# yoseph007/PQA2

Hardware: AMD Instinct MI355X
Metric: VMAF frames/sec (vif+adm+motion2 -> SVM), device-resident synthetic YUV pairs (higher is better)
Workload: dtype f32; 1 GPU; 2160p 3840x2160 8-bit, vmaf_4k_v0.6.1, 300 frames/GPU; frames_per_gpu=300, frames_total=300, batch=97, frames_per_launch=75, clips_pipelined=True, parallelism=frame-shard x1, 1-frame motion halo, all-gather of records + of scores

## Files before the change

pqa2_amd/csrc/kernels.h:

```cpp
#pragma once
#include <hip/hip_runtime.h>
#include <stdint.h>

namespace pqa {

enum Elem : int { ELEM_U8 = 0, ELEM_U16 = 1, ELEM_F32 = 2 };

struct PlaneRun {
  const void* base;
  int64_t row_pitch;
  int64_t frame_pitch;
};

struct MutPlaneRun {
  void* base;
  int64_t row_pitch;
  int64_t frame_pitch;
};

int vif_tile_w(int scale);
constexpr int kVifTileH = 8;
inline int vif_tiles_x(int scale, int w) { return (w + vif_tile_w(scale) - 1) / vif_tile_w(scale); }
inline int vif_tiles_y(int h) { return (h + kVifTileH - 1) / kVifTileH; }

enum : int { VIF_S0_VALU = 0, VIF_S0_AUTO = 1 };
hipError_t launch_vif_stat(hipStream_t stream, int scale, Elem elem, PlaneRun ref, PlaneRun dis, int n_frames,
                           int w, int h, float inv_scale, float gain_limit, int border101, double* partials,
                           MutPlaneRun next_ref, MutPlaneRun next_dis, int s0_mode = VIF_S0_AUTO, int* n_partials = nullptr);
hipError_t vif_march_prepare();
int vif_march_partials_max(int w, int h);
int vif_march_table(uint16_t* out, int capacity_halfwords);
void vif_march_shape(int w, int h, int* out6);
bool launch_vif_s0_march(hipStream_t stream, Elem elem, int bits, PlaneRun ref, PlaneRun dis, int n_frames, int w, int h, float gain_limit,
                         int border101, double* partials, MutPlaneRun next_ref, MutPlaneRun next_dis, int* n_partials,
                         hipError_t* err);
constexpr int kVifFxPartials = 8;
void vif_fixed_log2_table(uint16_t* out32768);
hipError_t launch_vif_fixed(hipStream_t stream, int scale, int bit_depth, Elem elem, PlaneRun ref, PlaneRun dis,
                            int n_frames, int w, int h, double gain_limit, const uint16_t* log2_lut,
                            long long* partials, MutPlaneRun next_ref, MutPlaneRun next_dis);

constexpr int kAdmTileW = 60, kAdmTileH = 14;
inline int adm_tiles_x(int band_w) { return (band_w + kAdmTileW - 1) / kAdmTileW; }
inline int adm_tiles_y(int band_h) { return (band_h + kAdmTileH - 1) / kAdmTileH; }

enum : int { ADM_TILED = 0, ADM_AUTO = 1, ADM_MARCH = 2 };
hipError_t launch_adm_scale(hipStream_t stream, int scale, Elem elem, PlaneRun ref, PlaneRun dis, int n_frames,
                            int w, int h, float inv_scale, float gain_limit, MutPlaneRun ll_ref,
                            MutPlaneRun ll_dis, double* partials, int mode = ADM_AUTO, int* n_partials = nullptr);
int adm_march_partials(int band_w, int band_h);
bool launch_adm_march(hipStream_t stream, int scale, Elem elem, PlaneRun ref, PlaneRun dis, int n_frames, int w, int h,
                      float inv_scale, float gain_limit, MutPlaneRun ll_ref, MutPlaneRun ll_dis, double* partials,
                      int* n_partials, hipError_t* err);
bool adm_pyramid_takes(Elem elem, int w, int h);
int adm_pyramid_partials(int w, int h);
bool launch_adm_pyramid(hipStream_t stream, Elem elem, PlaneRun ref, PlaneRun dis, int n_frames, int w, int h, float inv_scale,
                        float gain_limit, MutPlaneRun ll_ref, MutPlaneRun ll_dis, double* partials0, double* partials1,
                        int* n_partials, hipError_t* err);
float adm_dwt_quant_step(int lambda, int theta);

constexpr int kAdmFxRows = kAdmTileH + 2;
// ... 110 lines not shown
```

pqa2_amd/csrc/pqa_api.hip:

```cpp
#include "../../include/pqa_vmaf.h"

#include <algorithm>
#include <atomic>
#include <condition_variable>
#include <cstdarg>
#include <cstdio>
#include <cstdlib>
#include <cstring>
#include <memory>
#include <mutex>
#include <string>
#include <thread>
#include <vector>

#include <cerrno>
#include <unistd.h>

#include "host_pack.h"
#include "host_ring.h"
#include "ingest.h"
#include "kernels.h"

using namespace pqa;
using pqa::host::PackPool;
// ... 103 lines not shown
  uint8_t* luma_dev[2] = {nullptr, nullptr};
  hipEvent_t luma_copied[2] = {nullptr, nullptr};
  int64_t luma_pitch = 0;
  int LB = 0;
  bool luma_ready = false;
  uint32_t luma_gray = PQA_GRAY_LUMA;
  uint8_t* last_luma = nullptr;
  int64_t last_luma_pitch = 0;
  int64_t last_index = -1;
  bool have_last = false, halo_armed = false;
  Half half[2];
  int cur_half = 0, pending = 0;
  int64_t pending_first = 0;
  size_t slot_bytes = 0;
  size_t plane_off[2][3] = {};
  int64_t slot_row_pitch[3] = {};
  bool staging_ready = false;
  std::thread pin_thread;
  hipError_t pin_err = hipSuccess;
  uint8_t* surf_dev = nullptr;
  std::unique_ptr<PackPool> pack_pool;
  bool pack_pool_tried = false;
  std::vector<PackTask> pack_tasks;
  host::RecordRing ring;
  hipEvent_t batch_ev[kBatchEvents] = {};
  uint64_t batch_ev_seq[kBatchEvents] = {};
  uint64_t batch_seq = 0;
  uint64_t done_seq = 0;
  std::atomic<int> cancelled{0};
  std::string err;
  std::vector<void*> allocs;
  int multi_stream = 0;
  int vif_s0_mode = VIF_S0_AUTO;
  int adm_mode = ADM_AUTO;
  int motion_mode = MOTION_AUTO;
  bool trace = false;
  bool prof = false;
  uint32_t prof_mask = 0xffffffffu;
  std::vector<ProfEv> evs;
  double prof_ms[PQA_PROF_KERNELS] = {};
  uint64_t prof_n[PQA_PROF_KERNELS] = {}, prof_frames[PQA_PROF_KERNELS] = {};
};

namespace {

int fail(pqa_ctx* c, int code, const char* fmt, ...) {
  char buf[512];
  va_list ap;
  va_start(ap, fmt);
  vsnprintf(buf, sizeof buf, fmt, ap);
  va_end(ap);
  if (c) c->err = buf; else g_create_error = buf;
  return code;
}

#define HIPCHK(c, expr)                                                                          \
  do {                                                                                           \
    hipError_t e_ = (expr);                                                                      \
    if (e_ != hipSuccess)                                                                        \
      return fail((c), e_ == hipErrorOutOfMemory ? PQA_ENOMEM : PQA_EDEVICE, "%s failed: %s", #expr, \
                  hipGetErrorString(e_));                                                        \
  } while (0)

template <typename T>
int dev_alloc(pqa_ctx* c, T** out, size_t count) {
  void* p = nullptr;
// ... 134 lines not shown
      if (s < 3) {
        Level& L = c->vif_lv[s + 1];
        nr = MutPlaneRun{L.ref, L.pitch, L.frame_pitch};
        nd = MutPlaneRun{L.dis, L.pitch, L.frame_pitch};
      }
      {
        ProfScope ps(c, s, sp_n, st);
        HIPCHK(c, launch_vif_fixed(st, s, (int)c->cfg.bit_depth, ce, cr, cd, sp_n, cw, ch, c->cfg.vif_enhn_gain_limit,
                                   c->vif_lut, c->vif_fx_part[s], nr, nd));
      }
      if (s < 3) {
        Level& L = c->vif_lv[s + 1];
        cr = PlaneRun{L.ref, L.pitch, L.frame_pitch};
        cd = PlaneRun{L.dis, L.pitch, L.frame_pitch};
        ce = ELEM_U16;
        cw = L.w; ch = L.h;
      }
    }
  } else if ((feat & PQA_FEAT_VIF) && sp_n > 0) {
    PlaneRun cr = rYs, cd = dYs;
    Elem ce = c->elem;
    int cw = w, ch = h;
    for (int s = 0; s < 4; ++s) {
      MutPlaneRun nr{nullptr, 0, 0}, nd{nullptr, 0, 0};
      if (s < 3) {
        Level& L = c->vif_lv[s + 1];
        nr = MutPlaneRun{L.ref, L.pitch, L.frame_pitch};
        nd = MutPlaneRun{L.dis, L.pitch, L.frame_pitch};
      }
      {
        ProfScope ps(c, s, sp_n, st);
        HIPCHK(c, launch_vif_stat(st, s, ce, cr, cd, sp_n, cw, ch, c->inv_scale,
                                  (float)c->cfg.vif_enhn_gain_limit, c->cfg.vif_border == PQA_VIF_BORDER_INTEGER,
                                  c->vif_part[s], nr, nd, c->vif_s0_mode, &vif_np[s]));
      }
      if (s == 0 && fork_late) {
        HIPCHK(c, hipEventRecord(c->fork_ev, st));
        HIPCHK(c, hipStreamWaitEvent(st_adm, c->fork_ev, 0));
        HIPCHK(c, hipStreamWaitEvent(st_misc, c->fork_ev, 0));
      }
      if (s < 3) {
        Level& L = c->vif_lv[s + 1];
        cr = PlaneRun{L.ref, L.pitch, L.frame_pitch};
        cd = PlaneRun{L.dis, L.pitch, L.frame_pitch};
        ce = ELEM_F32;
        cw = L.w; ch = L.h;
      }
    }
  }
  if ((feat & PQA_FEAT_ADM) && sp_n > 0 && c->adm_fixed) {
    PlaneRun cr = rYs, cd = dYs;
    Elem ce = c->elem;
    int cw = w, ch = h;
    for (int s = 0; s < 4; ++s) {
      MutPlaneRun lr{nullptr, 0, 0}, ld{nullptr, 0, 0};
      if (s < 3) {
        Level& L = c->adm_lv[s + 1];
        lr = MutPlaneRun{L.ref, L.pitch, L.frame_pitch};
        ld = MutPlaneRun{L.dis, L.pitch, L.frame_pitch};
      }
      {
        ProfScope ps(c, 7 + s, sp_n, st_adm);
        HIPCHK(c, launch_adm_fixed(st_adm, s, (int)c->cfg.bit_depth, ce, cr, cd, sp_n, cw, ch,
                                   c->cfg.adm_enhn_gain_limit, c->adm_div_lut, lr, ld, c->adm_fx_part[s]));
      }
      if (s < 3) {
        Level& L = c->adm_lv[s + 1];
// ... 534 lines not shown
  c->k_sub = cfg->n_subsample > 1 ? (int)cfg->n_subsample : 1;
  if (c->cfg.vif_enhn_gain_limit <= 0) c->cfg.vif_enhn_gain_limit = 100.0;
  if (c->cfg.adm_enhn_gain_limit <= 0) c->cfg.adm_enhn_gain_limit = 100.0;
  c->elem = cfg->bit_depth > 8 ? ELEM_U16 : ELEM_U8;
  c->esize = cfg->bit_depth > 8 ? 2 : 1;
  c->inv_scale = 1.0f / (float)(1 << (cfg->bit_depth - 8));
  c->n_planes = (int)cfg->n_planes;
  c->pw[0] = (int)cfg->width; c->ph[0] = (int)cfg->height;
  for (int p = 1; p < 3; ++p) {
    c->pw[p] = (int)((cfg->width + (1u << cfg->chroma_hshift) - 1) >> cfg->chroma_hshift);
    c->ph[p] = (int)((cfg->height + (1u << cfg->chroma_vshift) - 1) >> cfg->chroma_vshift);
  }

  auto bail = [&](int rc) {
    g_create_error = c->err;
    pqa_destroy(c);
    return rc;
  };
#define CREATE_TRY(expr) do { int rc_ = (expr); if (rc_ != PQA_OK) return bail(rc_); } while (0)
#define CREATE_HIP(expr) do { hipError_t e_ = (expr); if (e_ != hipSuccess) { \
    fail(c, e_ == hipErrorOutOfMemory ? PQA_ENOMEM : PQA_EDEVICE, "%s failed: %s", #expr, hipGetErrorString(e_)); \
    return bail(e_ == hipErrorOutOfMemory ? PQA_ENOMEM : PQA_EDEVICE); } } while (0)

  CREATE_HIP(hipSetDevice(c->device));
  CREATE_HIP(hipStreamCreateWithFlags(&c->own_stream, hipStreamNonBlocking));
  c->stream = c->own_stream;
  {
    const char* e = getenv("PQA_MULTI_STREAM");
    c->multi_stream = (e && e[0] == '1') ? 1 : (e && e[0] == '2') ? 2 : 0;
    const char* t = getenv("PQA_TRACE");
    c->trace = t && t[0] == '1';
    const char* v = getenv("PQA_VIF_MFMA");
    c->vif_s0_mode = (v && v[0] == '0') ? VIF_S0_VALU : VIF_S0_AUTO;
    const char* am = getenv("PQA_ADM_MARCH");
    const char* ap = getenv("PQA_ADM_PYRAMID");
    c->adm_mode = (am && am[0] == '0') ? ADM_TILED : (ap && ap[0] == '0') ? ADM_MARCH : ADM_AUTO;
    const char* mm = getenv("PQA_MOTION_MARCH");
    c->motion_mode = (mm && mm[0] == '0') ? MOTION_TILED : MOTION_AUTO;
  }
  for (int i = 0; i < 2; ++i) {
    CREATE_HIP(hipStreamCreateWithFlags(&c->aux[i], hipStreamNonBlocking));
    CREATE_HIP(hipEventCreateWithFlags(&c->join_ev[i], hipEventDisableTiming));
  }
  CREATE_HIP(hipEventCreateWithFlags(&c->fork_ev, hipEventDisableTiming));
  for (int i = 0; i < kBatchEvents; ++i) CREATE_HIP(hipEventCreateWithFlags(&c->batch_ev[i], hipEventDisableTiming));
  try {
    c->ring.init(c->capacity);
  } catch (...) {
    fail(c, PQA_ENOMEM, "out of host memory");
    return bail(PQA_ENOMEM);
  }

  c->vif_fixed = (cfg->features & PQA_FEAT_VIF) && (cfg->fixed_point & PQA_FIXED_VIF);
  c->motion_fixed = (cfg->features & PQA_FEAT_MOTION) && (cfg->fixed_point & PQA_FIXED_MOTION);
  c->adm_fixed = (cfg->features & PQA_FEAT_ADM) && (cfg->fixed_point & PQA_FIXED_ADM);
  if (c->adm_fixed) {
    std::vector<int32_t> lut(65537);
    adm_fixed_div_table(lut.data());
    CREATE_TRY(dev_alloc(c, &c->adm_div_lut, lut.size()));
    CREATE_HIP(hipMemcpy(c->adm_div_lut, lut.data(), lut.size() * sizeof(int32_t), hipMemcpyHostToDevice));
  }
  if ((cfg->features & PQA_FEAT_VIF) && !c->vif_fixed) CREATE_HIP(vif_march_prepare());
  if (c->vif_fixed) {
    std::vector<uint16_t> lut(32768);
    vif_fixed_log2_table(lut.data());
    CREATE_TRY(dev_alloc(c, &c->vif_lut, lut.size()));
    CREATE_HIP(hipMemcpy(c->vif_lut, lut.data(), lut.size() * sizeof(uint16_t), hipMemcpyHostToDevice));
  }
  const int w = c->pw[0], h = c->ph[0], B = c->B;
  int vw = w, vh = h, aw = w, ah = h;
  for (int s = 0; s < 4; ++s) {
    if (s > 0) {
      vw /= 2; vh /= 2;
      aw = (aw + 1) / 2; ah = (ah + 1) / 2;
      Level& V = c->vif_lv[s];
      V.w = vw; V.h = vh; V.pitch = round_up(vw, 16); V.frame_pitch = V.pitch * vh;
      Level& A = c->adm_lv[s];
      A.w = aw; A.h = ah; A.pitch = round_up(aw, 16); A.frame_pitch = A.pitch * ah;
      if (cfg->features & PQA_FEAT_VIF) {
        CREATE_TRY(dev_alloc(c, &V.ref, (size_t)V.frame_pitch * B));
        CREATE_TRY(dev_alloc(c, &V.dis, (size_t)V.frame_pitch * B));
      }
      if (cfg->features & PQA_FEAT_ADM) {
        CREATE_TRY(dev_alloc(c, &A.ref, (size_t)A.frame_pitch * B));
        CREATE_TRY(dev_alloc(c, &A.dis, (size_t)A.frame_pitch * B));
      }
    }
    if (vw < 2 || vh < 2) { fail(c, PQA_EINVAL, "frame too small for 4 VIF scales"); return bail(PQA_EINVAL); }
    c->vif_tiles[s] = vif_tiles_x(s, vw) * vif_tiles_y(vh);
    if (s == 0) {
      const int mp = vif_march_partials_max(vw, vh);
      c->vif_part_cap0 = c->vif_tiles[0] > mp ? c->vif_tiles[0] : mp;
    }
    const int bw = (aw + 1) / 2, bh = (ah + 1) / 2;
    c->adm_tiles[s] = adm_tiles_x(bw) * adm_tiles_y(bh);
    const int left = (int)(bw * 0.1 - 0.5), top = (int)(bh * 0.1 - 0.5);
    c->adm_area[s] = (float)((bh - 2 * top) * (bw - 2 * left));
    if ((cfg->features & PQA_FEAT_VIF) && !c->vif_fixed)
      CREATE_TRY(dev_alloc(c, &c->vif_part[s], (size_t)(s == 0 ? c->vif_part_cap0 : c->vif_tiles[s]) * 2 * B));
    if ((cfg->features & PQA_FEAT_VIF) && c->vif_fixed)
      CREATE_TRY(dev_alloc(c, &c->vif_fx_part[s], (size_t)c->vif_tiles[s] * kVifFxPartials * B));
    c->adm_fx[s] = adm_fixed_scale_params(s, bw, bh);
    if ((cfg->features & PQA_FEAT_ADM) && !c->adm_fixed) {
      int mp = adm_march_partials(bw, bh);
      if (s < 2 && adm_pyramid_takes(c->elem, w, h)) { const int pp = adm_pyramid_partials(w, h); mp = pp > mp ? pp : mp; }
      CREATE_TRY(dev_alloc(c, &c->adm_part[s], (size_t)(c->adm_tiles[s] > mp ? c->adm_tiles[s] : mp) * 6 * B));
    }
    if ((cfg->features & PQA_FEAT_ADM) && c->adm_fixed)
      CREATE_TRY(dev_alloc(c, &c->adm_fx_part[s], (size_t)c->adm_tiles[s] * kAdmFxRows * 6 * B));
  }
  c->motion_tiles_n = motion_tiles(w, h);
  if (cfg->features & PQA_FEAT_MOTION) {
    {
      const int mp = motion_march_partials(w, h);
      CREATE_TRY(dev_alloc(c, &c->motion_part, (size_t)(c->motion_tiles_n > mp ? c->motion_tiles_n : mp) * B));
    }
    if (c->motion_fixed) CREATE_TRY(dev_alloc(c, &c->motion_fx_part, (size_t)c->motion_tiles_n * B));
    c->last_luma_pitch = round_up((int64_t)w * c->esize, 64);
    CREATE_TRY(dev_alloc(c, &c->last_luma, (size_t)c->last_luma_pitch * h));
  }
  for (int p = 0; p < c->n_planes; ++p) {
    if (cfg->features & PQA_FEAT_PSNR) {
      CREATE_TRY(dev_alloc(c, &c->sse_part[p], (size_t)kSseBlocksPerPlane * B));
      CREATE_TRY(dev_alloc(c, &c->sse_part_b[p], (size_t)kSseBlocksPerPlane * B));
    }
    if (cfg->features & PQA_FEAT_SSIM) {
      c->ssim_tiles_n[p] = ssim_tiles(c->pw[p], c->ph[p]);
      const int ww = (c->pw[p] >> 2) - 1, wh = (c->ph[p] >> 2) - 1;
      c->ssim_norm[p] = (ww > 0 && wh > 0) ? 1.0 / ((double)ww * wh) : 0.0;
      CREATE_TRY(dev_alloc(c, &c->ssim_part[p], (size_t)(c->ssim_tiles_n[p] ? c->ssim_tiles_n[p] : 1) * B));
      CREATE_TRY(dev_alloc(c, &c->sse_tile_part[p], (size_t)(c->ssim_tiles_n[p] ? c->ssim_tiles_n[p] : 1) * B));
    }
// ... 578 lines not shown
```

pqa2_amd/csrc/vif.hip:

```cpp
#include <cstring>
#include <mutex>
#include <vector>

#include <cstdio>
#include "kernels.h"
#include "pqa_device.h"

namespace pqa {

namespace {

struct Taps {
  float f[17];
};

static Taps gaussian_taps(int n) {
  Taps t{};
  double v[17], sum = 0.0;
  const double sigma = n / 5.0;
  for (int k = 0; k < n; ++k) {
    const double d = k - n / 2;
    v[k] = exp(-0.5 * d * d / (sigma * sigma));
    sum += v[k];
  }
  for (int k = 0; k < n; ++k) t.f[k] = (float)(v[k] / sum);
  return t;
}

struct TapPairs {
  f2 vt[18];
  f2 ht[17];
  f2 dt[9];
};

static TapPairs tap_pairs(const Taps& t, int n, const Taps* next, int n_next) {
  TapPairs p{};
  if (next)
    for (int k = 0; k < n_next; ++k) p.dt[k] = f2{next->f[k], next->f[k]};
  for (int k = 0; k <= n; ++k) {
    p.vt[k].x = k < n ? t.f[k] : 0.0f;
    p.vt[k].y = k > 0 ? t.f[k - 1] : 0.0f;
  }
  for (int k = 0; k < n; ++k) p.ht[k] = f2{t.f[k], t.f[k]};
  return p;
}

struct VifStatArgs {
  const void* ref;
  const void* dis;
  int64_t row_pitch_r, frame_pitch_r, row_pitch_d, frame_pitch_d;
  int w, h, tiles_x, n_tiles;
  int fold_w, fold_h;
  float inv_scale, gain_limit;
  double* partials;
  float* dst_ref;
  float* dst_dis;
  int64_t dst_row_pitch_r, dst_frame_pitch_r, dst_row_pitch_d, dst_frame_pitch_d;
  TapPairs taps;
};

constexpr int kP2 = 258;


template <int N, int TW, int ND>
__device__ __forceinline__ void vif_hstat(const VifStatArgs& a, const f2* sv ,
                                          const f2* sd , double* red, int fr, int tile, int x0, int y0) {
  constexpr int R = N / 2, TH = kVifTileH, NSEG = TW / 4, NRP = TH / 2;
  constexpr int RD = ND / 2;
  const int tid = threadIdx.x;
  fr = __builtin_amdgcn_readfirstlane(fr); tile = __builtin_amdgcn_readfirstlane(tile);
  x0 = __builtin_amdgcn_readfirstlane(x0); y0 = __builtin_amdgcn_readfirstlane(y0);
  if (ND) {
    const int ox0 = x0 >> 1, oy0 = y0 >> 1, ow = a.w >> 1, oh = a.h >> 1;
    float* __restrict__ tr = a.dst_ref + ((int64_t)fr * a.dst_frame_pitch_r + (int64_t)oy0 * a.dst_row_pitch_r + ox0);
    float* __restrict__ td = a.dst_dis + ((int64_t)fr * a.dst_frame_pitch_d + (int64_t)oy0 * a.dst_row_pitch_d + ox0);
    const unsigned rp_r = (unsigned)a.dst_row_pitch_r, rp_d = (unsigned)a.dst_row_pitch_d;
#pragma unroll
    for (int round = 0; round < 2; ++round) {
      const int item = tid + round * kBlock;
      const int oc = item & 127, orow = item >> 7;
      if (oc < TW / 2 && (ox0 + oc < ow && oy0 + orow < oh)) {
        f2 acc = f2{0.0f, 0.0f};
#pragma unroll
        for (int k = 0; k < ND; ++k) acc = __builtin_elementwise_fma(a.taps.dt[k], sd[orow * kP2 + 2 * oc + (R - RD) + k], acc);
        *reinterpret_cast<float*>(reinterpret_cast<char*>(tr) + ((unsigned)orow * rp_r + (unsigned)oc) * 4u) = acc.x;
        *reinterpret_cast<float*>(reinterpret_cast<char*>(td) + ((unsigned)orow * rp_d + (unsigned)oc) * 4u) = acc.y;
      }
    }
  }

  const int wave = tid >> 6, lane = tid & 63;
  const int rp = lane & 3, sl = lane >> 2;
  const int seg = 2 * (sl & 3) + (wave & 1) + 8 * (sl >> 2) + 32 * (wave >> 1);
  float num = 0.0f, den = 0.0f;
  if (seg < NSEG) {
    constexpr int NCOL = 4 + N - 1, NREAD = (NCOL + 1) / 2;
    f2 out[5][4];
#pragma unroll
    for (int s = 0; s < 5; ++s) {
      f2 in[2 * NREAD];
      const f4* p = reinterpret_cast<const f4*>(&sv[(s * NRP + rp) * kP2 + seg * 4]);
#pragma unroll
      for (int q = 0; q < NREAD; ++q) {
        const f4 v = p[q];
        in[2 * q] = f2{v.x, v.y};
        in[2 * q + 1] = f2{v.z, v.w};
      }
#pragma unroll
      for (int o = 0; o < 4; ++o) out[s][o] = f2{0.0f, 0.0f};
#pragma unroll
      for (int k = 0; k < N; ++k)
#pragma unroll
        for (int o = 0; o < 4; ++o) out[s][o] = __builtin_elementwise_fma(a.taps.ht[k], in[o + k], out[s][o]);
      __builtin_amdgcn_sched_barrier(0);
    }
    const float sigma_nsq = 2.0f, eps = 1.0e-10f, sigma_max_inv = 4.0f / (255.0f * 255.0f);
    const int gyA = y0 + 2 * rp;
    const bool vrow[2] = {gyA < a.h, gyA + 1 < a.h};
    f2 num2 = f2{0.0f, 0.0f}, den2 = f2{0.0f, 0.0f};
    f2 pn = f2{1.0f, 1.0f}, qn = f2{1.0f, 1.0f}, pd = f2{1.0f, 1.0f};
#pragma unroll
    for (int o = 0; o < 4; ++o) {
      const bool vcol = (x0 + seg * 4 + o) < a.w;
      const f2 mu1 = out[0][o], mu2 = out[1][o];
      const f2 s1 = out[2][o] - mu1 * mu1;
      f2 s2 = out[3][o] - mu2 * mu2;
      const f2 s12 = out[4][o] - mu1 * mu2;
      s2 = f2{fmaxf(s2.x, 0.0f), fmaxf(s2.y, 0.0f)};
      const bool vx = vcol && vrow[0], vy = vcol && vrow[1];
      const bool hx = vx && !(s1.x < sigma_nsq), hy = vy && !(s1.y < sigma_nsq);
      const bool lx = vx && (s1.x < sigma_nsq), ly = vy && (s1.y < sigma_nsq);
      const f2 s1h = f2{hx ? s1.x : 0.0f, hy ? s1.y : 0.0f};
      const f2 gden = s1h + f2{eps, eps};
      const f2 grcp = f2{fast_rcp(gden.x), fast_rcp(gden.y)};
      f2 g = s12 * grcp;
      g = __builtin_elementwise_fma(__builtin_elementwise_fma(-g, gden, s12), grcp, g);
      f2 sv = s2 - g * s12;
      sv = f2{fmaxf(sv.x, eps), fmaxf(sv.y, eps)};
      g = f2{__builtin_amdgcn_fmed3f(g.x, 0.0f, a.gain_limit), __builtin_amdgcn_fmed3f(g.y, 0.0f, a.gain_limit)};
      const f2 svn = sv + f2{sigma_nsq, sigma_nsq};
      const f2 narg = __builtin_elementwise_fma(g * g, s1h, svn);
      const f2 darg = __builtin_elementwise_fma(s1h, f2{1.0f / sigma_nsq, 1.0f / sigma_nsq}, f2{1.0f, 1.0f});
      const f2 low = __builtin_elementwise_fma(s2, f2{-sigma_max_inv, -sigma_max_inv}, f2{1.0f, 1.0f});
      pn *= narg;
      qn *= svn;
      pd *= darg;
      const f2 wl = f2{lx ? 1.0f : 0.0f, ly ? 1.0f : 0.0f};
      num2 = __builtin_elementwise_fma(wl, low, num2);
      den2 += wl;
      __builtin_amdgcn_sched_barrier(0);
    }
    num = (num2.x + num2.y) + ((fast_log2(pn.x) - fast_log2(qn.x)) + (fast_log2(pn.y) - fast_log2(qn.y)));
    den = (den2.x + den2.y) + (fast_log2(pd.x) + fast_log2(pd.y));
  }
  {
    const float part[2] = {num, den};
    double v[2];
    block_sum_f32<2>(part, v, red);
    if (tid == 0) {
      double* out = a.partials + ((int64_t)fr * a.n_tiles + tile) * 2;
      out[0] = v[0];
      out[1] = v[1];
    }
  }
}

template <typename T, int N, int TW, int ND>
__global__ __launch_bounds__(kBlock, 3) void vif_stat_kernel(const VifStatArgs a) {
  constexpr int R = N / 2, TH = kVifTileH, COLS = TW + N - 1, NSEG = TW / 4, S = 8, NIN = S + N - 1;
  constexpr int RD = ND / 2;
  static_assert(ND == 0 || RD <= R, "decimation window must sit inside the statistic window");
  static_assert(COLS <= 256 && COLS <= kP2, "one column per thread");
  static_assert(TW % 4 == 0 && NSEG <= 64 && TH == S, "segment map");
  __shared__ f2 sv[5][TH / 2][kP2];
  __shared__ f2 sd[ND ? TH / 2 : 1][ND ? kP2 : 1];
  __shared__ double red[12];

  const int tile = xcd_remap(blockIdx.x, a.n_tiles);
  const int tx = tile % a.tiles_x, ty = tile / a.tiles_x;
  const int fr = blockIdx.y;
  const T* __restrict__ ref = (const T*)a.ref + (int64_t)fr * a.frame_pitch_r;
  const T* __restrict__ dis = (const T*)a.dis + (int64_t)fr * a.frame_pitch_d;
  const int x0 = tx * TW, y0 = ty * TH;
  const int tid = threadIdx.x;

  {
    const int col = tid;
    constexpr int seg = 0;
    if (col < COLS) {
      const unsigned gx = (unsigned)mirror_fold(x0 - R + col, a.w, a.fold_w);
      const unsigned pitch_r = (unsigned)a.row_pitch_r, pitch_d = (unsigned)a.row_pitch_d;
      const auto rsrc_r = make_rsrc(ref, (unsigned)a.h * pitch_r * (unsigned)sizeof(T));
      const auto rsrc_d = make_rsrc(dis, (unsigned)a.h * pitch_d * (unsigned)sizeof(T));
      f2 acc[S / 2][5];
#pragma unroll
      for (int p = 0; p < S / 2; ++p)
// ... 61 lines not shown
        for (int s = 0; s < 5; ++s) sv[s][seg * (S / 2) + p][col] = acc[p][s];
      if (ND) {
#pragma unroll
        for (int q = 0; q < S / 2; ++q) sd[seg * (S / 2) + q][col] = dacc[q];
      }
    }
  }
  __syncthreads();

  vif_hstat<N, TW, ND>(a, &sv[0][0][0], &sd[0][0], red, fr, tile, x0, y0);
}


template <int N, int TW, int ND>
hipError_t launch_stat_n(hipStream_t stream, Elem elem, const VifStatArgs& a, int n_frames) {
  const dim3 grid(a.n_tiles, n_frames), block(kBlock);
  switch (elem) {
    case ELEM_U8: hipLaunchKernelGGL((vif_stat_kernel<uint8_t, N, TW, ND>), grid, block, 0, stream, a); break;
    case ELEM_U16: hipLaunchKernelGGL((vif_stat_kernel<uint16_t, N, TW, ND>), grid, block, 0, stream, a); break;
    case ELEM_F32: hipLaunchKernelGGL((vif_stat_kernel<float, N, TW, ND>), grid, block, 0, stream, a); break;
  }
  return hipGetLastError();
}

constexpr int kVifN[4] = {17, 9, 5, 3};
constexpr int kVifTW[4] = {240, 248, 252, 252};

}

int vif_tile_w(int scale) { return kVifTW[scale]; }

hipError_t launch_vif_stat(hipStream_t stream, int scale, Elem elem, PlaneRun ref, PlaneRun dis, int n_frames,
                           int w, int h, float inv_scale, float gain_limit, int border101, double* partials,
                           MutPlaneRun next_ref, MutPlaneRun next_dis, int s0_mode, int* n_partials) {
  if (n_partials) *n_partials = vif_tiles_x(scale, w) * vif_tiles_y(h);
  if (n_frames <= 0) return hipSuccess;
  const int bits = elem == ELEM_U8 ? 8 : (elem == ELEM_U16 && inv_scale == 0.25f) ? 10 : (elem == ELEM_U16 && inv_scale == 0.0625f) ? 12 : 0;
  if (scale == 0 && bits && s0_mode == VIF_S0_AUTO && next_ref.base && next_dis.base) {
    hipError_t err = hipSuccess;
    if (launch_vif_s0_march(stream, elem, bits, ref, dis, n_frames, w, h, gain_limit, border101, partials, next_ref, next_dis, n_partials, &err))
      return err;
    if (n_partials) *n_partials = vif_tiles_x(scale, w) * vif_tiles_y(h);
  }
  VifStatArgs a{};
  a.ref = ref.base; a.dis = dis.base;
  a.row_pitch_r = ref.row_pitch; a.frame_pitch_r = ref.frame_pitch;
  a.row_pitch_d = dis.row_pitch; a.frame_pitch_d = dis.frame_pitch;
  a.w = w; a.h = h;
  a.fold_w = 2 * w - (border101 ? 2 : 1); a.fold_h = 2 * h - (border101 ? 2 : 1);
  a.tiles_x = vif_tiles_x(scale, w);
  a.n_tiles = a.tiles_x * vif_tiles_y(h);
  a.inv_scale = inv_scale; a.gain_limit = gain_limit;
  a.partials = partials;
  a.dst_ref = (float*)next_ref.base; a.dst_dis = (float*)next_dis.base;
  a.dst_row_pitch_r = next_ref.row_pitch; a.dst_frame_pitch_r = next_ref.frame_pitch;
  a.dst_row_pitch_d = next_dis.row_pitch; a.dst_frame_pitch_d = next_dis.frame_pitch;
  const Taps cur = gaussian_taps(kVifN[scale]);
  const Taps nxt = scale < 3 ? gaussian_taps(kVifN[scale + 1]) : Taps{};
  a.taps = tap_pairs(cur, kVifN[scale], scale < 3 ? &nxt : nullptr, scale < 3 ? kVifN[scale + 1] : 0);
  if (scale < 3 && (!a.dst_ref || !a.dst_dis)) return hipErrorInvalidValue;
  switch (scale) {
    case 0: return launch_stat_n<17, 240, 9>(stream, elem, a, n_frames);
    case 1: return launch_stat_n<9, 248, 5>(stream, elem, a, n_frames);
    case 2: return launch_stat_n<5, 252, 3>(stream, elem, a, n_frames);
    case 3: return launch_stat_n<3, 252, 0>(stream, elem, a, n_frames);
  }
  return hipErrorInvalidValue;
}

}
```

Before: 22040 frames/s.

## Add tall-tile VIF kernel for scales 1-2 reusing vertical halo across chunks

Adds a VIF statistic kernel for scales 1 and 2 that processes 32-row tiles as four 8-row chunks. Vertical filter accumulators carry over between chunks, so the N-1 halo rows are not reloaded and recomputed for every 8-row tile. It also prefetches the next chunk's rows while the current chunk runs. The shared horizontal-stat and decimation code moves into a common header, and the partial buffers are sized for the new tile count. The cost is fewer blocks, which lowers parallelism at the smaller scales, plus more registers for the carried accumulators.

```diff
diff --git a/pqa2_amd/csrc/kernels.h b/pqa2_amd/csrc/kernels.h
--- a/pqa2_amd/csrc/kernels.h
+++ b/pqa2_amd/csrc/kernels.h
@@ -23,10 +23,12 @@
 inline int vif_tiles_x(int scale, int w) { return (w + vif_tile_w(scale) - 1) / vif_tile_w(scale); }
 inline int vif_tiles_y(int h) { return (h + kVifTileH - 1) / kVifTileH; }
 
+int vif_tall_tiles(int scale, int w, int h);
 enum : int { VIF_S0_VALU = 0, VIF_S0_AUTO = 1 };
 hipError_t launch_vif_stat(hipStream_t stream, int scale, Elem elem, PlaneRun ref, PlaneRun dis, int n_frames,
                            int w, int h, float inv_scale, float gain_limit, int border101, double* partials,
-                           MutPlaneRun next_ref, MutPlaneRun next_dis, int s0_mode = VIF_S0_AUTO, int* n_partials = nullptr);
+                           MutPlaneRun next_ref, MutPlaneRun next_dis, int s0_mode = VIF_S0_AUTO, int* n_partials = nullptr,
+                           int tall = 1);
 hipError_t vif_march_prepare();
 int vif_march_partials_max(int w, int h);
 int vif_march_table(uint16_t* out, int capacity_halfwords);
diff --git a/pqa2_amd/csrc/pqa_api.hip b/pqa2_amd/csrc/pqa_api.hip
--- a/pqa2_amd/csrc/pqa_api.hip
+++ b/pqa2_amd/csrc/pqa_api.hip
@@ -159,6 +159,7 @@
   std::vector<void*> allocs;
   int multi_stream = 0;
   int vif_s0_mode = VIF_S0_AUTO;
+  int vif_tall = 1;
   int adm_mode = ADM_AUTO;
   int motion_mode = MOTION_AUTO;
   bool trace = false;
@@ -359,7 +360,7 @@
         ProfScope ps(c, s, sp_n, st);
         HIPCHK(c, launch_vif_stat(st, s, ce, cr, cd, sp_n, cw, ch, c->inv_scale,
                                   (float)c->cfg.vif_enhn_gain_limit, c->cfg.vif_border == PQA_VIF_BORDER_INTEGER,
-                                  c->vif_part[s], nr, nd, c->vif_s0_mode, &vif_np[s]));
+                                  c->vif_part[s], nr, nd, c->vif_s0_mode, &vif_np[s], c->vif_tall));
       }
       if (s == 0 && fork_late) {
         HIPCHK(c, hipEventRecord(c->fork_ev, st));
@@ -960,6 +961,8 @@
     c->trace = t && t[0] == '1';
     const char* v = getenv("PQA_VIF_MFMA");
     c->vif_s0_mode = (v && v[0] == '0') ? VIF_S0_VALU : VIF_S0_AUTO;
+    const char* vt = getenv("PQA_VIF_TALL");
+    c->vif_tall = !(vt && vt[0] == '0');
     const char* am = getenv("PQA_ADM_MARCH");
     const char* ap = getenv("PQA_ADM_PYRAMID");
     c->adm_mode = (am && am[0] == '0') ? ADM_TILED : (ap && ap[0] == '0') ? ADM_MARCH : ADM_AUTO;
@@ -1024,8 +1027,10 @@
     c->adm_tiles[s] = adm_tiles_x(bw) * adm_tiles_y(bh);
     const int left = (int)(bw * 0.1 - 0.5), top = (int)(bh * 0.1 - 0.5);
     c->adm_area[s] = (float)((bh - 2 * top) * (bw - 2 * left));
-    if ((cfg->features & PQA_FEAT_VIF) && !c->vif_fixed)
-      CREATE_TRY(dev_alloc(c, &c->vif_part[s], (size_t)(s == 0 ? c->vif_part_cap0 : c->vif_tiles[s]) * 2 * B));
+    if ((cfg->features & PQA_FEAT_VIF) && !c->vif_fixed) {
+      const int cap = s == 0 ? c->vif_part_cap0 : (c->vif_tiles[s] > vif_tall_tiles(s, vw, vh) ? c->vif_tiles[s] : vif_tall_tiles(s, vw, vh));
+      CREATE_TRY(dev_alloc(c, &c->vif_part[s], (size_t)cap * 2 * B));
+    }
     if ((cfg->features & PQA_FEAT_VIF) && c->vif_fixed)
       CREATE_TRY(dev_alloc(c, &c->vif_fx_part[s], (size_t)c->vif_tiles[s] * kVifFxPartials * B));
     c->adm_fx[s] = adm_fixed_scale_params(s, bw, bh);
diff --git a/pqa2_amd/csrc/vif.hip b/pqa2_amd/csrc/vif.hip
--- a/pqa2_amd/csrc/vif.hip
+++ b/pqa2_amd/csrc/vif.hip
@@ -5,163 +5,26 @@
 #include <cstdio>
 #include "kernels.h"
 #include "pqa_device.h"
+#include "vif_common.h"
 
 namespace pqa {
 
 namespace {
 
-struct Taps {
-  float f[17];
-};
-
-static Taps gaussian_taps(int n) {
-  Taps t{};
-  double v[17], sum = 0.0;
-  const double sigma = n / 5.0;
-  for (int k = 0; k < n; ++k) {
-    const double d = k - n / 2;
-    v[k] = exp(-0.5 * d * d / (sigma * sigma));
-    sum += v[k];
-  }
-  for (int k = 0; k < n; ++k) t.f[k] = (float)(v[k] / sum);
-  return t;
-}
-
-struct TapPairs {
-  f2 vt[18];
-  f2 ht[17];
-  f2 dt[9];
-};
-
-static TapPairs tap_pairs(const Taps& t, int n, const Taps* next, int n_next) {
-  TapPairs p{};
-  if (next)
-    for (int k = 0; k < n_next; ++k) p.dt[k] = f2{next->f[k], next->f[k]};
-  for (int k = 0; k <= n; ++k) {
-    p.vt[k].x = k < n ? t.f[k] : 0.0f;
-    p.vt[k].y = k > 0 ? t.f[k - 1] : 0.0f;
-  }
-  for (int k = 0; k < n; ++k) p.ht[k] = f2{t.f[k], t.f[k]};
-  return p;
-}
-
-struct VifStatArgs {
-  const void* ref;
-  const void* dis;
-  int64_t row_pitch_r, frame_pitch_r, row_pitch_d, frame_pitch_d;
-  int w, h, tiles_x, n_tiles;
-  int fold_w, fold_h;
-  float inv_scale, gain_limit;
-  double* partials;
-  float* dst_ref;
-  float* dst_dis;
-  int64_t dst_row_pitch_r, dst_frame_pitch_r, dst_row_pitch_d, dst_frame_pitch_d;
-  TapPairs taps;
-};
-
-constexpr int kP2 = 258;
-
-
 template <int N, int TW, int ND>
 __device__ __forceinline__ void vif_hstat(const VifStatArgs& a, const f2* sv ,
                                           const f2* sd , double* red, int fr, int tile, int x0, int y0) {
-  constexpr int R = N / 2, TH = kVifTileH, NSEG = TW / 4, NRP = TH / 2;
-  constexpr int RD = ND / 2;
-  const int tid = threadIdx.x;
   fr = __builtin_amdgcn_readfirstlane(fr); tile = __builtin_amdgcn_readfirstlane(tile);
   x0 = __builtin_amdgcn_readfirstlane(x0); y0 = __builtin_amdgcn_readfirstlane(y0);
-  if (ND) {
-    const int ox0 = x0 >> 1, oy0 = y0 >> 1, ow = a.w >> 1, oh = a.h >> 1;
-    float* __restrict__ tr = a.dst_ref + ((int64_t)fr * a.dst_frame_pitch_r + (int64_t)oy0 * a.dst_row_pitch_r + ox0);
-    float* __restrict__ td = a.dst_dis + ((int64_t)fr * a.dst_frame_pitch_d + (int64_t)oy0 * a.dst_row_pitch_d + ox0);
-    const unsigned rp_r = (unsigned)a.dst_row_pitch_r, rp_d = (unsigned)a.dst_row_pitch_d;
-#pragma unroll
-    for (int round = 0; round < 2; ++round) {
-      const int item = tid + round * kBlock;
-      const int oc = item & 127, orow = item >> 7;
-      if (oc < TW / 2 && (ox0 + oc < ow && oy0 + orow < oh)) {
-        f2 acc = f2{0.0f, 0.0f};
-#pragma unroll
-        for (int k = 0; k < ND; ++k) acc = __builtin_elementwise_fma(a.taps.dt[k], sd[orow * kP2 + 2 * oc + (R - RD) + k], acc);
-        *reinterpret_cast<float*>(reinterpret_cast<char*>(tr) + ((unsigned)orow * rp_r + (unsigned)oc) * 4u) = acc.x;
-        *reinterpret_cast<float*>(reinterpret_cast<char*>(td) + ((unsigned)orow * rp_d + (unsigned)oc) * 4u) = acc.y;
-      }
-    }
-  }
-
-  const int wave = tid >> 6, lane = tid & 63;
-  const int rp = lane & 3, sl = lane >> 2;
-  const int seg = 2 * (sl & 3) + (wave & 1) + 8 * (sl >> 2) + 32 * (wave >> 1);
-  float num = 0.0f, den = 0.0f;
-  if (seg < NSEG) {
-    constexpr int NCOL = 4 + N - 1, NREAD = (NCOL + 1) / 2;
-    f2 out[5][4];
-#pragma unroll
-    for (int s = 0; s < 5; ++s) {
-      f2 in[2 * NREAD];
-      const f4* p = reinterpret_cast<const f4*>(&sv[(s * NRP + rp) * kP2 + seg * 4]);
-#pragma unroll
-      for (int q = 0; q < NREAD; ++q) {
-        const f4 v = p[q];
-        in[2 * q] = f2{v.x, v.y};
-        in[2 * q + 1] = f2{v.z, v.w};
-      }
-#pragma unroll
-      for (int o = 0; o < 4; ++o) out[s][o] = f2{0.0f, 0.0f};
-#pragma unroll
-      for (int k = 0; k < N; ++k)
-#pragma unroll
-        for (int o = 0; o < 4; ++o) out[s][o] = __builtin_elementwise_fma(a.taps.ht[k], in[o + k], out[s][o]);
-      __builtin_amdgcn_sched_barrier(0);
-    }
-    const float sigma_nsq = 2.0f, eps = 1.0e-10f, sigma_max_inv = 4.0f / (255.0f * 255.0f);
-    const int gyA = y0 + 2 * rp;
-    const bool vrow[2] = {gyA < a.h, gyA + 1 < a.h};
-    f2 num2 = f2{0.0f, 0.0f}, den2 = f2{0.0f, 0.0f};
-    f2 pn = f2{1.0f, 1.0f}, qn = f2{1.0f, 1.0f}, pd = f2{1.0f, 1.0f};
-#pragma unroll
-    for (int o = 0; o < 4; ++o) {
-      const bool vcol = (x0 + seg * 4 + o) < a.w;
-      const f2 mu1 = out[0][o], mu2 = out[1][o];
-      const f2 s1 = out[2][o] - mu1 * mu1;
-      f2 s2 = out[3][o] - mu2 * mu2;
-      const f2 s12 = out[4][o] - mu1 * mu2;
-      s2 = f2{fmaxf(s2.x, 0.0f), fmaxf(s2.y, 0.0f)};
-      const bool vx = vcol && vrow[0], vy = vcol && vrow[1];
-      const bool hx = vx && !(s1.x < sigma_nsq), hy = vy && !(s1.y < sigma_nsq);
-      const bool lx = vx && (s1.x < sigma_nsq), ly = vy && (s1.y < sigma_nsq);
-      const f2 s1h = f2{hx ? s1.x : 0.0f, hy ? s1.y : 0.0f};
-      const f2 gden = s1h + f2{eps, eps};
-      const f2 grcp = f2{fast_rcp(gden.x), fast_rcp(gden.y)};
-      f2 g = s12 * grcp;
-      g = __builtin_elementwise_fma(__builtin_elementwise_fma(-g, gden, s12), grcp, g);
-      f2 sv = s2 - g * s12;
-      sv = f2{fmaxf(sv.x, eps), fmaxf(sv.y, eps)};
-      g = f2{__builtin_amdgcn_fmed3f(g.x, 0.0f, a.gain_limit), __builtin_amdgcn_fmed3f(g.y, 0.0f, a.gain_limit)};
-      const f2 svn = sv + f2{sigma_nsq, sigma_nsq};
-      const f2 narg = __builtin_elementwise_fma(g * g, s1h, svn);
-      const f2 darg = __builtin_elementwise_fma(s1h, f2{1.0f / sigma_nsq, 1.0f / sigma_nsq}, f2{1.0f, 1.0f});
-      const f2 low = __builtin_elementwise_fma(s2, f2{-sigma_max_inv, -sigma_max_inv}, f2{1.0f, 1.0f});
-      pn *= narg;
-      qn *= svn;
-      pd *= darg;
-      const f2 wl = f2{lx ? 1.0f : 0.0f, ly ? 1.0f : 0.0f};
-      num2 = __builtin_elementwise_fma(wl, low, num2);
-      den2 += wl;
-      __builtin_amdgcn_sched_barrier(0);
-    }
-    num = (num2.x + num2.y) + ((fast_log2(pn.x) - fast_log2(qn.x)) + (fast_log2(pn.y) - fast_log2(qn.y)));
-    den = (den2.x + den2.y) + (fast_log2(pd.x) + fast_log2(pd.y));
-  }
-  {
-    const float part[2] = {num, den};
-    double v[2];
-    block_sum_f32<2>(part, v, red);
-    if (tid == 0) {
-      double* out = a.partials + ((int64_t)fr * a.n_tiles + tile) * 2;
-      out[0] = v[0];
-      out[1] = v[1];
-    }
+  vif_decimate_chunk<N, TW, ND>(a, sd, fr, x0, y0, threadIdx.x);
+  float part[2];
+  vif_hstat_chunk<N, TW>(a, sv, x0, y0, threadIdx.x, part[0], part[1]);
+  double v[2];
+  block_sum_f32<2>(part, v, red);
+  if (threadIdx.x == 0) {
+    double* out = a.partials + ((int64_t)fr * a.n_tiles + tile) * 2;
+    out[0] = v[0];
+    out[1] = v[1];
   }
 }
 
@@ -289,8 +152,9 @@
 
 hipError_t launch_vif_stat(hipStream_t stream, int scale, Elem elem, PlaneRun ref, PlaneRun dis, int n_frames,
                            int w, int h, float inv_scale, float gain_limit, int border101, double* partials,
-                           MutPlaneRun next_ref, MutPlaneRun next_dis, int s0_mode, int* n_partials) {
-  if (n_partials) *n_partials = vif_tiles_x(scale, w) * vif_tiles_y(h);
+                           MutPlaneRun next_ref, MutPlaneRun next_dis, int s0_mode, int* n_partials, int tall) {
+  tall = tall && (scale == 1 || scale == 2) && elem == ELEM_F32;
+  if (n_partials) *n_partials = tall ? vif_tall_tiles(scale, w, h) : vif_tiles_x(scale, w) * vif_tiles_y(h);
   if (n_frames <= 0) return hipSuccess;
   const int bits = elem == ELEM_U8 ? 8 : (elem == ELEM_U16 && inv_scale == 0.25f) ? 10 : (elem == ELEM_U16 && inv_scale == 0.0625f) ? 12 : 0;
   if (scale == 0 && bits && s0_mode == VIF_S0_AUTO && next_ref.base && next_dis.base) {
@@ -316,6 +180,7 @@
   const Taps nxt = scale < 3 ? gaussian_taps(kVifN[scale + 1]) : Taps{};
   a.taps = tap_pairs(cur, kVifN[scale], scale < 3 ? &nxt : nullptr, scale < 3 ? kVifN[scale + 1] : 0);
   if (scale < 3 && (!a.dst_ref || !a.dst_dis)) return hipErrorInvalidValue;
+  if (tall) return launch_vif_tall(stream, scale, a, n_frames);
   switch (scale) {
     case 0: return launch_stat_n<17, 240, 9>(stream, elem, a, n_frames);
     case 1: return launch_stat_n<9, 248, 5>(stream, elem, a, n_frames);
diff --git a/pqa2_amd/csrc/vif_common.h b/pqa2_amd/csrc/vif_common.h
--- /dev/null
+++ b/pqa2_amd/csrc/vif_common.h
@@ -0,0 +1,160 @@
+#pragma once
+#include <cmath>
+
+#include "kernels.h"
+#include "pqa_device.h"
+
+namespace pqa {
+
+struct Taps {
+  float f[17];
+};
+
+static Taps gaussian_taps(int n) {
+  Taps t{};
+  double v[17], sum = 0.0;
+  const double sigma = n / 5.0;
+  for (int k = 0; k < n; ++k) {
+    const double d = k - n / 2;
+    v[k] = exp(-0.5 * d * d / (sigma * sigma));
+    sum += v[k];
+  }
+  for (int k = 0; k < n; ++k) t.f[k] = (float)(v[k] / sum);
+  return t;
+}
+
+struct TapPairs {
+  f2 vt[18];
+  f2 ht[17];
+  f2 dt[9];
+};
+
+static TapPairs tap_pairs(const Taps& t, int n, const Taps* next, int n_next) {
+  TapPairs p{};
+  if (next)
+    for (int k = 0; k < n_next; ++k) p.dt[k] = f2{next->f[k], next->f[k]};
+  for (int k = 0; k <= n; ++k) {
+    p.vt[k].x = k < n ? t.f[k] : 0.0f;
+    p.vt[k].y = k > 0 ? t.f[k - 1] : 0.0f;
+  }
+  for (int k = 0; k < n; ++k) p.ht[k] = f2{t.f[k], t.f[k]};
+  return p;
+}
+
+struct VifStatArgs {
+  const void* ref;
+  const void* dis;
+  int64_t row_pitch_r, frame_pitch_r, row_pitch_d, frame_pitch_d;
+  int w, h, tiles_x, n_tiles;
+  int fold_w, fold_h;
+  float inv_scale, gain_limit;
+  double* partials;
+  float* dst_ref;
+  float* dst_dis;
+  int64_t dst_row_pitch_r, dst_frame_pitch_r, dst_row_pitch_d, dst_frame_pitch_d;
+  TapPairs taps;
+};
+
+constexpr int kP2 = 258;
+
+
+template <int N, int TW, int ND>
+__device__ __forceinline__ void vif_decimate_chunk(const VifStatArgs& a, const f2* sd , int fr, int x0, int y0,
+                                                   int tid ) {
+  constexpr int R = N / 2;
+  constexpr int RD = ND / 2;
+  if (ND) {
+    const int ox0 = x0 >> 1, oy0 = y0 >> 1, ow = a.w >> 1, oh = a.h >> 1;
+    float* __restrict__ tr = a.dst_ref + ((int64_t)fr * a.dst_frame_pitch_r + (int64_t)oy0 * a.dst_row_pitch_r + ox0);
+    float* __restrict__ td = a.dst_dis + ((int64_t)fr * a.dst_frame_pitch_d + (int64_t)oy0 * a.dst_row_pitch_d + ox0);
+    const unsigned rp_r = (unsigned)a.dst_row_pitch_r, rp_d = (unsigned)a.dst_row_pitch_d;
+#pragma unroll
+    for (int round = 0; round < 2; ++round) {
+      const int item = tid + round * kBlock;
+      const int oc = item & 127, orow = item >> 7;
+      if (oc < TW / 2 && (ox0 + oc < ow && oy0 + orow < oh)) {
+        f2 acc = f2{0.0f, 0.0f};
+#pragma unroll
+        for (int k = 0; k < ND; ++k) acc = __builtin_elementwise_fma(a.taps.dt[k], sd[orow * kP2 + 2 * oc + (R - RD) + k], acc);
+        *reinterpret_cast<float*>(reinterpret_cast<char*>(tr) + ((unsigned)orow * rp_r + (unsigned)oc) * 4u) = acc.x;
+        *reinterpret_cast<float*>(reinterpret_cast<char*>(td) + ((unsigned)orow * rp_d + (unsigned)oc) * 4u) = acc.y;
+      }
+    }
+  }
+}
+
+template <int N, int TW>
+__device__ __forceinline__ void vif_hstat_chunk(const VifStatArgs& a, const f2* sv , int x0, int y0,
+                                                int tid , float& num_out, float& den_out) {
+  constexpr int TH = kVifTileH, NSEG = TW / 4, NRP = TH / 2;
+  const int wave = tid >> 6, lane = tid & 63;
+  const int rp = lane & 3, sl = lane >> 2;
+  const int seg = 2 * (sl & 3) + (wave & 1) + 8 * (sl >> 2) + 32 * (wave >> 1);
+  float num = 0.0f, den = 0.0f;
+  if (seg < NSEG) {
+    constexpr int NCOL = 4 + N - 1, NREAD = (NCOL + 1) / 2;
+    f2 out[5][4];
+#pragma unroll
+    for (int s = 0; s < 5; ++s) {
+      f2 in[2 * NREAD];
+      const f4* p = reinterpret_cast<const f4*>(&sv[(s * NRP + rp) * kP2 + seg * 4]);
+#pragma unroll
+      for (int q = 0; q < NREAD; ++q) {
+        const f4 v = p[q];
+        in[2 * q] = f2{v.x, v.y};
+        in[2 * q + 1] = f2{v.z, v.w};
+      }
+#pragma unroll
+      for (int o = 0; o < 4; ++o) out[s][o] = f2{0.0f, 0.0f};
+#pragma unroll
+      for (int k = 0; k < N; ++k)
+#pragma unroll
+        for (int o = 0; o < 4; ++o) out[s][o] = __builtin_elementwise_fma(a.taps.ht[k], in[o + k], out[s][o]);
+      __builtin_amdgcn_sched_barrier(0);
+    }
+    const float sigma_nsq = 2.0f, eps = 1.0e-10f, sigma_max_inv = 4.0f / (255.0f * 255.0f);
+    const int gyA = y0 + 2 * rp;
+    const bool vrow[2] = {gyA < a.h, gyA + 1 < a.h};
+    f2 num2 = f2{0.0f, 0.0f}, den2 = f2{0.0f, 0.0f};
+    f2 pn = f2{1.0f, 1.0f}, qn = f2{1.0f, 1.0f}, pd = f2{1.0f, 1.0f};
+#pragma unroll
+    for (int o = 0; o < 4; ++o) {
+      const bool vcol = (x0 + seg * 4 + o) < a.w;
+      const f2 mu1 = out[0][o], mu2 = out[1][o];
+      const f2 s1 = out[2][o] - mu1 * mu1;
+      f2 s2 = out[3][o] - mu2 * mu2;
+      const f2 s12 = out[4][o] - mu1 * mu2;
+      s2 = f2{fmaxf(s2.x, 0.0f), fmaxf(s2.y, 0.0f)};
+      const bool vx = vcol && vrow[0], vy = vcol && vrow[1];
+      const bool hx = vx && !(s1.x < sigma_nsq), hy = vy && !(s1.y < sigma_nsq);
+      const bool lx = vx && (s1.x < sigma_nsq), ly = vy && (s1.y < sigma_nsq);
+      const f2 s1h = f2{hx ? s1.x : 0.0f, hy ? s1.y : 0.0f};
+      const f2 gden = s1h + f2{eps, eps};
+      const f2 grcp = f2{fast_rcp(gden.x), fast_rcp(gden.y)};
+      f2 g = s12 * grcp;
+      g = __builtin_elementwise_fma(__builtin_elementwise_fma(-g, gden, s12), grcp, g);
+      f2 sv = s2 - g * s12;
+      sv = f2{fmaxf(sv.x, eps), fmaxf(sv.y, eps)};
+      g = f2{__builtin_amdgcn_fmed3f(g.x, 0.0f, a.gain_limit), __builtin_amdgcn_fmed3f(g.y, 0.0f, a.gain_limit)};
+      const f2 svn = sv + f2{sigma_nsq, sigma_nsq};
+      const f2 narg = __builtin_elementwise_fma(g * g, s1h, svn);
+      const f2 darg = __builtin_elementwise_fma(s1h, f2{1.0f / sigma_nsq, 1.0f / sigma_nsq}, f2{1.0f, 1.0f});
+      const f2 low = __builtin_elementwise_fma(s2, f2{-sigma_max_inv, -sigma_max_inv}, f2{1.0f, 1.0f});
+      pn *= narg;
+      qn *= svn;
+      pd *= darg;
+      const f2 wl = f2{lx ? 1.0f : 0.0f, ly ? 1.0f : 0.0f};
+      num2 = __builtin_elementwise_fma(wl, low, num2);
+      den2 += wl;
+      __builtin_amdgcn_sched_barrier(0);
+    }
+    num = (num2.x + num2.y) + ((fast_log2(pn.x) - fast_log2(qn.x)) + (fast_log2(pn.y) - fast_log2(qn.y)));
+    den = (den2.x + den2.y) + (fast_log2(pd.x) + fast_log2(pd.y));
+  }
+  num_out = num;
+  den_out = den;
+}
+
+hipError_t launch_vif_tall(hipStream_t stream, int scale, const VifStatArgs& args, int n_frames);
+
+}
diff --git a/pqa2_amd/csrc/vif_tall.hip b/pqa2_amd/csrc/vif_tall.hip
--- /dev/null
+++ b/pqa2_amd/csrc/vif_tall.hip
@@ -0,0 +1,172 @@
+#include "kernels.h"
+#include "pqa_device.h"
+#include "vif_common.h"
+
+namespace pqa {
+
+namespace {
+
+#ifndef PQA_VIF_TALL_TH
+#define PQA_VIF_TALL_TH 32
+#endif
+constexpr int kTallTH = PQA_VIF_TALL_TH;
+constexpr int kTallS = 8;
+
+template <int N>
+__device__ __forceinline__ void tall_tap(const VifStatArgs& a, f2& acc, int k, float x) {
+  if (k == 0) acc = __builtin_elementwise_fma(a.taps.vt[0], f2{x, x}, f2{0.0f, 0.0f});
+  else if (k < N) acc = __builtin_elementwise_fma(a.taps.vt[k], f2{x, x}, acc);
+  else if (k == N) acc.y = __builtin_fmaf(a.taps.vt[N].y, x, acc.y);
+}
+
+struct TallSig {
+  float r, d, rr, dd, rd;
+};
+__device__ __forceinline__ TallSig tall_sig(float r, float d) {
+  const f2 xx = f2{r, d} * f2{r, d};
+  return TallSig{r, d, xx.x, xx.y, r * d};
+}
+
+template <int N, int ND, bool FIN>
+__device__ __forceinline__ void tall_row(const VifStatArgs& a, int jr, const TallSig& x, f2 (&acc)[kTallS / 2][5],
+                                         f2 (&dacc)[kTallS / 2]) {
+  constexpr int R = N / 2, RD = ND / 2, NP = kTallS / 2;
+  const int j = FIN ? jr : jr - kTallS;
+  if (ND) {
+#pragma unroll
+    for (int q = 0; q < NP; ++q) {
+      const int kd = j - (2 * q + R - RD);
+      if (kd >= 0 && kd < ND)
+        dacc[q] = __builtin_elementwise_fma(a.taps.dt[kd], f2{x.r, x.d}, kd == 0 ? f2{0.0f, 0.0f} : dacc[q]);
+    }
+  }
+#pragma unroll
+  for (int p = 0; p < NP; ++p) {
+    const int k = j - 2 * p;
+    if (k >= 0 && k <= N) {
+      tall_tap<N>(a, acc[p][0], k, x.r); tall_tap<N>(a, acc[p][1], k, x.d); tall_tap<N>(a, acc[p][2], k, x.rr);
+      tall_tap<N>(a, acc[p][3], k, x.dd); tall_tap<N>(a, acc[p][4], k, x.rd);
+    }
+  }
+}
+
+template <int N, int TW, int ND, int TH>
+__global__ __launch_bounds__(kBlock, 3) void vif_tall_kernel(const VifStatArgs a) {
+  constexpr int R = N / 2, COLS = TW + N - 1, S = kTallS, NP = S / 2, NCH = TH / S;
+  constexpr int RD = ND / 2;
+  static_assert(S == kVifTileH, "the shared phases take 8-row chunks");
+  static_assert(N - 1 <= S, "an input row reaches the current and the next chunk only");
+  static_assert(ND == 0 || RD <= R, "decimation window must sit inside the statistic window");
+  static_assert(COLS <= 256 && COLS <= kP2 && TW % 4 == 0 && TW / 4 <= 64, "one column per thread, segment map");
+  static_assert(TH % S == 0, "whole chunks");
+  __shared__ f2 sv[5][NP][kP2];
+  __shared__ f2 sd[ND ? NP : 1][ND ? kP2 : 1];
+  __shared__ double red[8];
+
+  const int tile = __builtin_amdgcn_readfirstlane(xcd_remap(blockIdx.x, a.n_tiles));
+  const int tx = tile % a.tiles_x, ty = tile / a.tiles_x;
+  const int fr = __builtin_amdgcn_readfirstlane((int)blockIdx.y);
+  const int x0 = __builtin_amdgcn_readfirstlane(tx * TW), y0 = __builtin_amdgcn_readfirstlane(ty * TH);
+  const int nch = __builtin_amdgcn_readfirstlane(min(NCH, (a.h - y0 + S - 1) / S));
+  const int tid = threadIdx.x;
+  const unsigned gx = (unsigned)mirror_fold(x0 - R + tid, a.w, a.fold_w);
+  const float* __restrict__ ref = (const float*)a.ref + (int64_t)fr * a.frame_pitch_r;
+  const float* __restrict__ dis = (const float*)a.dis + (int64_t)fr * a.frame_pitch_d;
+  const unsigned pitch_r = (unsigned)a.row_pitch_r, pitch_d = (unsigned)a.row_pitch_d;
+  const auto rsrc_r = make_rsrc(ref, (unsigned)a.h * pitch_r * 4u);
+  const auto rsrc_d = make_rsrc(dis, (unsigned)a.h * pitch_d * 4u);
+
+  float rn[S], dn[S];
+  auto issue = [&](int c) {
+#pragma unroll
+    for (int i = 0; i < S; ++i) {
+      const int j = c * S + N - 1 + i;
+      if (j >= 0) {
+        const unsigned gy = (unsigned)mirror_fold(y0 - R + j, a.h, a.fold_h);
+        rn[i] = buf_load<float>(rsrc_r, gx, gy * pitch_r);
+        dn[i] = buf_load<float>(rsrc_d, gx, gy * pitch_d);
+      }
+    }
+  };
+
+  f2 acc[NP][5], dacc[NP];
+  double numd = 0.0, dend = 0.0;
+
+  issue(-1);
+  {
+    TallSig x[S];
+#pragma unroll
+    for (int i = 0; i < S; ++i) x[i] = tall_sig(rn[i], dn[i]);
+    issue(0);
+#pragma unroll
+    for (int i = 0; i < S; ++i)
+      if (N - 1 + i - S >= 0) tall_row<N, ND, false>(a, N - 1 + i, x[i], acc, dacc);
+  }
+
+  for (int c = 0; c < nch; ++c) {
+    float rc[S], dc[S];
+#pragma unroll
+    for (int i = 0; i < S; ++i) { rc[i] = rn[i]; dc[i] = dn[i]; }
+    if (c + 1 < nch) issue(c + 1);
+#pragma unroll
+    for (int i = 0; i < S; ++i) tall_row<N, ND, true>(a, N - 1 + i, tall_sig(rc[i], dc[i]), acc, dacc);
+    __syncthreads();
+#pragma unroll
+    for (int p = 0; p < NP; ++p)
+#pragma unroll
+      for (int s = 0; s < 5; ++s) sv[s][p][tid] = acc[p][s];
+    if (ND) {
+#pragma unroll
+      for (int q = 0; q < NP; ++q) sd[q][tid] = dacc[q];
+    }
+    __syncthreads();
+    const int yc = __builtin_amdgcn_readfirstlane(y0 + c * S);
+    int t = tid;
+    asm volatile("" : "+v"(t));
+    vif_decimate_chunk<N, TW, ND>(a, &sd[0][0], fr, x0, yc, t);
+    float num, den;
+    vif_hstat_chunk<N, TW>(a, &sv[0][0][0], x0, yc, t, num, den);
+    numd += (double)num;
+    dend += (double)den;
+    if (c + 1 < nch) {
+#pragma unroll
+      for (int i = 0; i < S; ++i) {
+        asm volatile("" : "+v"(rc[i]), "+v"(dc[i]));
+        tall_row<N, ND, false>(a, N - 1 + i, tall_sig(rc[i], dc[i]), acc, dacc);
+      }
+    }
+  }
+
+  double v[2] = {numd, dend};
+  block_sum<2>(v, red);
+  if (tid == 0) {
+    double* out = a.partials + ((int64_t)fr * a.n_tiles + tile) * 2;
+    out[0] = v[0];
+    out[1] = v[1];
+  }
+}
+
+template <int N, int TW, int ND>
+hipError_t launch_tall_n(hipStream_t stream, const VifStatArgs& a, int n_frames) {
+  hipLaunchKernelGGL((vif_tall_kernel<N, TW, ND, kTallTH>), dim3(a.n_tiles, n_frames), dim3(kBlock), 0, stream, a);
+  return hipGetLastError();
+}
+
+}
+
+int vif_tall_tiles(int scale, int w, int h) {
+  return scale == 1 || scale == 2 ? vif_tiles_x(scale, w) * ((h + kTallTH - 1) / kTallTH) : 0;
+}
+
+hipError_t launch_vif_tall(hipStream_t stream, int scale, const VifStatArgs& args, int n_frames) {
+  VifStatArgs a = args;
+  a.tiles_x = vif_tiles_x(scale, a.w);
+  a.n_tiles = vif_tall_tiles(scale, a.w, a.h);
+  switch (scale) {
+    case 1: return launch_tall_n<9, 248, 5>(stream, a, n_frames);
+    case 2: return launch_tall_n<5, 252, 3>(stream, a, n_frames);
+  }
+  return hipErrorInvalidValue;
+}
+
+}
```

After: 22350 frames/s, median of 6. +1.4%, better.
